# Gericom/MobiclipDecoder

Measured on AMD Instinct MI355X. Metric: decoded Mpixels/s @ 640x480 P-frames, higher is better.
Workload: dtype u8

## Files before the change

### mobiclipdecoder_amd/csrc/mobi_kernels.hip

```cpp
#include <hip/hip_runtime.h>
#include <stdint.h>
#include <stdlib.h>

#include <type_traits>

#include "mobi_cmd.h"
#include "mobi_kernels.h"
#include "mobi_recon_math.h"
#include "mobi_tile.h"

namespace {

enum { TP = 32 };

__device__ __forceinline__ void wave_sync() { __builtin_amdgcn_fence(__ATOMIC_ACQ_REL, "wavefront"); }

struct Geo {
  int width, height, stride, mbw, lg;
  __device__ __forceinline__ int owner_luma(int a) const {
    if (a < 0) return -1;
    const int row = a >> lg, col = a & (stride - 1);
    if (col >= width || row >= height) return -1;
    return (row >> 4) * mbw + (col >> 4);
  }
// ... 121 lines not shown
#else
#define MOBI_STOP(n) do { } while (0)
#define MOBI_ISTOP(n) do { } while (0)
#endif
namespace {
typedef const void __attribute__((address_space(1))) *gptr_t;
typedef void __attribute__((address_space(3))) *lptr_t;
#define MOBI_DMA16(src, dst, IMM) __builtin_amdgcn_global_load_lds((gptr_t)(src), (lptr_t)(dst), 16, IMM, 0)
__device__ __forceinline__ void dma16_sv(const uint8_t *base, uint32_t voff, uint32_t lds) {
#if defined(__HIP_DEVICE_COMPILE__)
  asm volatile("s_mov_b32 m0, %2\n\ts_nop 0\n\tglobal_load_lds_dwordx4 %0, %1" : : "v"(voff), "s"(base), "s"(lds) : "memory", "m0");
#endif
}

__device__ __forceinline__ uint32_t lds32(const uint8_t *L, int byte_off) { return *(const uint32_t *)(L + byte_off); }
typedef short s16x2 __attribute__((ext_vector_type(2)));
__device__ __forceinline__ uint32_t sat_pk_u8(s16x2 v) {
#if defined(__HIP_DEVICE_COMPILE__)
  uint32_t d;
  asm("v_sat_pk_u8_i16 %0, %1" : "=v"(d) : "v"(v));
  return d;
#else
  const int a = v.x < 0 ? 0 : v.x > 255 ? 255 : v.x, b = v.y < 0 ? 0 : v.y > 255 ? 255 : v.y;
  return (uint32_t)a | ((uint32_t)b << 8);
#endif
}
__device__ __forceinline__ void idct_pass2_q(const int *t, bool is8, int r, uint8_t *wa, uint8_t *wb, s16x2 &lo, s16x2 &hi) {
  int in[8], out[8];
  if (is8) {
#pragma unroll
    for (int m = 0; m < 8; m++) in[m] = t[8 * r + m];
    mobi_bfly8(in, out);
  } else {
    const int s = r >> 1, i0 = (r & 1) * 2;
#pragma unroll
    for (int m = 0; m < 8; m++) in[m] = t[16 * s + 4 * i0 + m];
    mobi_bfly4(in, out);
    mobi_bfly4(in + 4, out + 4);
  }
  const uint32_t pw[2] = {*(const uint32_t *)wa, *(const uint32_t *)wb};
  uint32_t res[2];
#pragma unroll
  for (int h = 0; h < 2; h++) {
    union { s16x2 v; uint32_t u; } p01, p23;
    p01.u = __builtin_amdgcn_perm(0u, pw[h], 0x0c010c00u);
    p23.u = __builtin_amdgcn_perm(0u, pw[h], 0x0c030c02u);
    const s16x2 r01 = __builtin_amdgcn_cvt_pk_i16(out[4 * h], out[4 * h + 1]) >> (short)6, r23 = __builtin_amdgcn_cvt_pk_i16(out[4 * h + 2], out[4 * h + 3]) >> (short)6;
    const s16x2 s01 = __builtin_elementwise_add_sat(p01.v, r01), s23 = __builtin_elementwise_add_sat(p23.v, r23);
    lo = __builtin_elementwise_min(lo, __builtin_elementwise_min(s01, s23));
    hi = __builtin_elementwise_max(hi, __builtin_elementwise_max(s01, s23));
    res[h] = __builtin_amdgcn_perm(sat_pk_u8(s23), sat_pk_u8(s01), 0x05040100u);
  }
  *(uint32_t *)wa = res[0];
  *(uint32_t *)wb = res[1];
}
}

#define MOBI_PK_LIMIT 14000
namespace {
__device__ __forceinline__ void bfly8_pk(const s16x2 in[8], s16x2 out[8]) {
  const s16x2 a0 = in[0] + in[4], a1 = in[0] - in[4];
  const s16x2 a2 = in[2] + (in[6] >> (short)1), a3 = (in[2] >> (short)1) - in[6];
  const s16x2 e0 = a0 + a2, e1 = a1 + a3, e2 = a1 - a3, e3 = a0 - a2;
  const s16x2 b0 = in[1] + in[7] - in[3] - (in[3] >> (short)1);
  const s16x2 b1 = in[7] - in[1] + in[5] + (in[5] >> (short)1);
  const s16x2 b2 = in[5] - (in[7] + (in[7] >> (short)1)) - in[3];
  const s16x2 b3 = in[3] + in[5] + in[1] + (in[1] >> (short)1);
  const s16x2 o0 = b2 + (b3 >> (short)2), o3 = b3 - (b2 >> (short)2);
  const s16x2 o1 = b0 + (b1 >> (short)2), o2 = (b0 >> (short)2) - b1;
  out[0] = e0 + o3; out[7] = e0 - o3;
  out[1] = e1 + o2; out[6] = e1 - o2;
  out[2] = e2 + o1; out[5] = e2 - o1;
  out[3] = e3 + o0; out[4] = e3 - o0;
}
__device__ __forceinline__ void bfly4_pk(const s16x2 in[4], s16x2 out[4]) {
  const s16x2 a = in[0] + in[2], b = in[0] - in[2];
  const s16x2 c = (in[1] >> (short)1) - in[3], d = in[1] + (in[3] >> (short)1);
  out[0] = a + d; out[3] = a - d; out[1] = b + c; out[2] = b - c;
}
union PkRow { uint4 q[2]; s16x2 v[8]; };
__device__ __forceinline__ void idct_pass1_pk(uint32_t *c, bool is8, int r) {
  PkRow in;
  s16x2 out[8];
  in.q[0] = *(const uint4 *)(c + 8 * r);
  in.q[1] = *(const uint4 *)(c + 8 * r + 4);
  const s16x2 rnd = {32, 32};
  if (is8) {
    if (r == 0) in.v[0] += rnd;
    bfly8_pk(in.v, out);
    wave_sync();
#pragma unroll
    for (int m = 0; m < 8; m++) *(s16x2 *)(c + 8 * m + r) = out[m];
  } else {
    const int s = r >> 1, k0 = (r & 1) * 2;
    if (k0 == 0) in.v[0] += rnd;
    bfly4_pk(in.v, out);
    bfly4_pk(in.v + 4, out + 4);
    wave_sync();
#pragma unroll
    for (int m = 0; m < 4; m++) *(uint2 *)(c + 16 * s + 4 * m + k0) = uint2{__builtin_bit_cast(uint32_t, out[m]), __builtin_bit_cast(uint32_t, out[4 + m])};
  }
}
__device__ __forceinline__ void idct_pass2_pk(const uint32_t *t, bool is8, int r, uint8_t *waA, uint8_t *wbA, uint8_t *waB, uint8_t *wbB, bool actB,
                                              s16x2 &lo, s16x2 &hi) {
  PkRow in;
  s16x2 out[8];
  in.q[0] = *(const uint4 *)(t + 8 * r);
  in.q[1] = *(const uint4 *)(t + 8 * r + 4);
  if (is8) {
    bfly8_pk(in.v, out);
  } else {
    bfly4_pk(in.v, out);
    bfly4_pk(in.v + 4, out + 4);
  }
  const uint32_t pA[2] = {*(const uint32_t *)waA, *(const uint32_t *)wbA}, pB[2] = {*(const uint32_t *)waB, *(const uint32_t *)wbB};
  uint32_t resA[2], resB[2];
#pragma unroll
  for (int h = 0; h < 2; h++) {
    uint32_t sat[4];
#pragma unroll
    for (int k = 0; k < 4; k++) {
      const s16x2 pp = __builtin_bit_cast(s16x2, __builtin_amdgcn_perm(pB[h], pA[h], 0x0c040c00u + (uint32_t)k * 0x00010001u));
      const s16x2 sum = __builtin_elementwise_add_sat(pp, out[4 * h + k] >> (short)6);
      lo = __builtin_elementwise_min(lo, sum);
      hi = __builtin_elementwise_max(hi, sum);
      sat[k] = sat_pk_u8(sum);
    }
    const uint32_t m01 = __builtin_amdgcn_perm(sat[1], sat[0], 0x05010400u), m23 = __builtin_amdgcn_perm(sat[3], sat[2], 0x05010400u);
    resA[h] = __builtin_amdgcn_perm(m23, m01, 0x05040100u);
    resB[h] = __builtin_amdgcn_perm(m23, m01, 0x07060302u);
  }
  *(uint32_t *)waA = resA[0];
  *(uint32_t *)wbA = resA[1];
  if (actB) {
    *(uint32_t *)waB = resB[0];
    *(uint32_t *)wbB = resB[1];
  }
}
}

namespace {
enum {
  P_L = 0,
  P_C = 5120,
  P_C1 = 7680,
  P_BYTES = 10240,
  P_OUT = 0,
  P_PITCH = 400,
  P_COEF = 3200,
  P_TILE = 72,
#ifndef MOBI_PK_PAIRS
#define MOBI_PK_PAIRS 12
#endif
  P_PAIRS = MOBI_PK_PAIRS,
  P_ROUND = 22,
  P_SUM = P_COEF + P_PAIRS * P_TILE * 4,
  P_SC = 9728,
  P_TAB = 10048,
  P_INV = 9536
};
static_assert(P_OUT + 7 * P_PITCH + 384 <= P_COEF && P_COEF + P_ROUND * P_TILE * 4 <= P_INV && P_INV + 192 <= P_SC && P_SC + 320 <= P_TAB && P_TAB + 192 <= P_BYTES && P_SUM + 192 <= P_INV, "inter LDS map");
static_assert(23 * P_TILE * 4 + 2 < (1 << 13) && (P_PITCH & 15) == 0, "P_INV's offset field (48 slots); 16-byte reads of the output rows");
__device__ __forceinline__ int out_px(int g, int R, int c) { return P_OUT + (R & 7) * P_PITCH + (R >> 3) * 128 + (g << 4) + c; }
__device__ __forceinline__ int out_y(int g, int R, int c) { return out_px(g, R, c); }
__device__ __forceinline__ int out_c(int g, int R, int pl, int x) { return out_px(g, 16 + R, pl * 8 + x); }
template <int N>
__device__ __forceinline__ void mc_rows(const uint32_t (&x0)[N + 1], const uint32_t (&x1)[N + 1], uint32_t sh, int phase, uint32_t *out) {
  const bool hor = (phase & 1) != 0, ver = (phase & 2) != 0;
  const uint32_t selA = 0x03020100u + sh * 0x01010101u, selB = hor ? selA + 0x01010101u : selA;
  const uint32_t Mh = hor ? 0xFEFEFEFEu : 0xFFFFFFFFu, Mv = ver ? 0xFEFEFEFEu : 0xFFFFFFFFu;
  uint32_t m[N + 1];
#pragma unroll
  for (int i = 0; i <= N; i++) {
    const uint32_t a = __builtin_amdgcn_perm(x1[i], x0[i], selA) & Mh, b = __builtin_amdgcn_perm(x1[i], x0[i], selB) & Mh;
    m[i] = __builtin_amdgcn_lerp(a, b, 0u) & Mv;
  }
#pragma unroll
  for (int i = 0; i < N; i++) out[i] = __builtin_amdgcn_lerp(m[i], ver ? m[i + 1] : m[i], 0u);
}
}

__device__ __forceinline__ unsigned long long prof_stamp() {
  __builtin_amdgcn_sched_barrier(0);
  asm volatile("" ::: "memory");
  const unsigned long long t = __builtin_readcyclecounter();
  asm volatile("" ::: "memory");
  __builtin_amdgcn_sched_barrier(0);
  return t;
}
template <int PROF, int CWR, int FUSED>
__device__ __forceinline__ void recon_inter_oct(const MobiReconArgs &A, uint8_t *L, uint32_t clip, uint32_t mby, uint32_t ox, int lane) {
  unsigned long long pt[7] = {0, 0, 0, 0, 0, 0, 0};
  if (PROF) pt[0] = prof_stamp();
  const uint32_t oi = clip * A.qpc + mby * A.qpr + ox;
  const uint32_t mbx0 = ox * 8, mbw = (uint32_t)A.mbw;
  const int nmb = (int)(mbw - mbx0 < 8 ? mbw - mbx0 : 8);
  const int S = A.stride, lgS = 31 - __builtin_clz((unsigned)S);
  const uint32_t ysz = (uint32_t)S * (uint32_t)A.height;
  uint8_t *clip_base = A.planes + (size_t)clip * A.clip_bytes;
  const uint32_t lds0 = (uint32_t)(size_t)(lptr_t)L;
  const int off0 = (int)(mby * 16 * (uint32_t)S + mbx0 * 16);
  const int g = lane & 7, j = lane >> 3;
  unsigned long long pa = 0, pb = 0;
  if (PROF) { asm volatile("" : : "s"(off0), "s"(clip)); pa = prof_stamp(); }

  __builtin_amdgcn_s_setprio(3);
  const uint4 *dp = (const uint4 *)(A.desc + (clip * (uint32_t)A.n_mbs + mby * mbw + mbx0) + g);
  const uint4 d = dp[0], d2 = dp[1];
  if (PROF) { asm volatile("s_waitcnt vmcnt(0)" ::: "memory"); pb = prof_stamp(); }
  const bool valid = g < nmb && (d.y & 1) == MOBI_MB_INTER;
  const int nl = (d.y >> 1) & 0x7F, kind2 = (d.y >> 26) & 3;
  const bool leaves = valid && (nl == 1 || kind2 != 0);
  const bool multi = valid && nl > 1 && kind2 == 0;
  const bool tb = leaves && kind2 == MOBI_DUAL_TB, lr = leaves && kind2 == MOBI_DUAL_LR;
  const uint32_t cbp6 = valid ? (d.y >> 8) & 0x3F : 0, ncoef = cbp6 ? d.z & 0x3FF : 0;
  const unsigned long long v64 = __builtin_amdgcn_ballot_w64(g < nmb) & __builtin_amdgcn_ballot_w64((d.y & 1) == MOBI_MB_INTER);
  const unsigned long long six = 0x0000FFFFFFFFFFFFull;
  const unsigned long long mb64 = __builtin_amdgcn_ballot_w64(((d.y >> (8 + j)) & 1) != 0) & v64 & six;
  const unsigned long long tb64 = __builtin_amdgcn_ballot_w64(((d.y >> (14 + j)) & 1) != 0) & six;
  const uint32_t m_lo = (uint32_t)mb64, m_hi = (uint32_t)(mb64 >> 32), t_lo = (uint32_t)tb64, t_hi = (uint32_t)(tb64 >> 32);
  const uint32_t inter_mask = (uint32_t)v64 & 0xFFu;
  const uint32_t multi_mask = (uint32_t)(v64 & __builtin_amdgcn_ballot_w64(nl > 1) & __builtin_amdgcn_ballot_w64(kind2 == 0)) & 0xFFu;
  if (inter_mask == 0) return;
  auto slot_off = [&](uint32_t ref) {
    int sl = A.ring_base - (int)ref;
    sl = sl < 0 ? sl + 6 : sl;
    return __umul24((uint32_t)sl, A.slot_bytes);
  };
  const uint32_t refA = slot_off((d.z >> 10) & 7), refB = slot_off((d.z >> 13) & 7);
  const int posA = (int)d.w, cposA = (int)d2.x, posB = (int)d2.y, cposB = (int)d2.z;
  const int phA = (d.z >> 16) & 3, cphA = (d.z >> 18) & 3, phB = (d.z >> 20) & 3, cphB = (d.z >> 22) & 3;
  const int topB = tb ? posB + (8 << lgS) : posB + 8, ctopB = tb ? cposB + (4 << lgS) : cposB + 4;
  const int wpx = lr ? 8 : 16, cwpx = lr ? 4 : 8;
  const int overA = max((posA & (S - 1)) + wpx + (phA & 1) - S, (cposA & (S - 1)) + cwpx + (cphA & 1) - (S >> 1));
  const int overB = max((topB & (S - 1)) + wpx + (phB & 1) - S, (ctopB & (S - 1)) + cwpx + (cphB & 1) - (S >> 1));
  const bool wrap = leaves && max(overA, kind2 != 0 ? overB : 0) > 0;
  const bool win = leaves && !wrap;
  const bool slow = multi || wrap;
  const uint32_t slow_mask = (uint32_t)__builtin_amdgcn_ballot_w64(slow) & 0xFFu;
  const bool any_lr = __builtin_amdgcn_ballot_w64(lr && win) != 0;
  {
    const int s = j & 3, ph = j >> 2;
    const bool colB = lr && s >= 2;
    const int sw = lr ? s & 1 : (s < 3 ? s : 2);
    auto chunk0 = [&](int top, uint32_t ref, uint32_t &u) {
      const int yo = (top >> lgS) & 1;
      const uint32_t lin = (uint32_t)(((top - (yo << lgS)) & ~7) + 8 * sw);
      u = lin >> (lgS + 1);
      return ref + mobi_ty_col(lin & (uint32_t)(S - 1));
    };
    uint32_t uP, uB;
    const uint32_t bP = chunk0(colB ? topB : posA, colB ? refB : refA, uP), bB = chunk0(topB, refB, uB);
    auto rowpart = [&](uint32_t v) { return ((v & ~7u) << (lgS + 1)) + (((v & 7u) + (v & 4u)) << 4); };
    const uint32_t Tm = (16u << lgS) - 256u;
    auto rows3 = [&](uint32_t base, uint32_t v, uint32_t (&r)[3]) {
      uint32_t h = (v >> 2) & 1u, e = (v >> 1) & 1u;
      asm volatile("" : "+v"(h), "+v"(e));
      const uint32_t dm = __umul24(h, Tm) + 64u;
      r[0] = base + rowpart(v);
      r[1] = __umul24(e, dm) + r[0] + 32u;
      r[2] = r[0] + 64u + dm;
    };
    const uint32_t vP = uP + (uint32_t)ph;
    uint32_t r1[3], r2[3];
    rows3(bP, vP, r1);
    rows3(tb ? bB : bP, tb ? uB + 1u - (uint32_t)ph : vP + 4u, r2);
    const bool early = tb && !ph;
    const bool short2 = tb != (ph != 0);
    const uint32_t o[5] = {r1[0], r1[1], early ? r1[2] : r2[0], early ? r2[0] : r2[1], short2 ? r2[1] : r2[2]};
    if (win) {
#pragma unroll
      for (int t = 0; t < 5; t++) dma16_sv(clip_base, o[t], lds0 + P_L + t * 1024);
    }
    const int cs = j & 1, ch2 = j >> 1;
    auto cchunk0 = [&](int ctop, uint32_t ref, uint32_t &r) {
      const uint32_t lin = (uint32_t)((ctop & ~7) + 8 * cs);
      r = lin >> lgS;
      return ref + ysz + mobi_tc_x(lin & (uint32_t)(S - 1));
    };
    auto crowpart = [&](uint32_t r) { return ((r & ~7u) << lgS) + ((r & 7u) << 4); };
    uint32_t rA, rB;
    const uint32_t cA = cchunk0(cposA, refA, rA), cB = cchunk0(ctopB, refB, rB);
    const uint32_t Tc = 8u << lgS, Tcm = Tc - 128u;
    auto cstep4 = [&](uint32_t r) {
      uint32_t h = (r >> 2) & 1u;
      asm volatile("" : "+v"(h));
      return __umul24(h, Tcm) + 64u;
    };
    const uint32_t qA = rA + (uint32_t)ch2;
    const uint32_t c0 = cA + crowpart(qA), cE = c0 + cstep4(qA);
    const uint32_t cY = cB + crowpart(rB + (uint32_t)((ch2 + 3) & 3));
    const uint32_t stB = cstep4(rB);
    const uint32_t cYd = cY + (ch2 == 1 ? stB : 0u);
    const uint32_t co[3] = {c0, (tb && ch2) ? cY : cE, tb ? cYd : (ch2 ? cE : c0 + Tc)};
    if (win) {
#pragma unroll
      for (int t = 0; t < 3; t++) dma16_sv(clip_base, co[t], lds0 + P_C + t * 1024);
    }
    if (any_lr) {
      const uint32_t q3 = rB + (uint32_t)ch2;
      if (lr && win) {
        const uint32_t z0 = cB + crowpart(q3), z1 = z0 + cstep4(q3);
        dma16_sv(clip_base, z0, lds0 + P_C1);
        dma16_sv(clip_base, z1, lds0 + P_C1 + 1024);
        dma16_sv(clip_base, ch2 ? z1 : z0 + Tc, lds0 + P_C1 + 2048);
      }
    }
  }
  MOBI_STOP(1);
  const int quant = __builtin_amdgcn_readfirstlane((int)((d.y >> 20) & 63));
  const uint32_t *pay = A.payload + (size_t)clip * A.pay_clip_words;
  const uint32_t *cw = pay + d.x + (multi ? MOBI_MV_CELLS : 0);
  uint32_t cwr[CWR];
#pragma unroll
  for (int k = 0; k < CWR; k++) asm volatile("" : "=v"(cwr[k]));
  const uint32_t *cwj = cw + j;
  const int left = (int)ncoef - j;
  if (left > 0) cwr[0] = cwj[0];
  if (__builtin_amdgcn_ballot_w64(ncoef > 8) != 0) {
#pragma unroll
    for (int k = 1; k < 4; k++)
      if (left > 8 * k) cwr[k] = cwj[8 * k];
    if (CWR > 4 && __builtin_amdgcn_ballot_w64(ncoef > 32) != 0) {
#pragma unroll
      for (int k = 4; k < CWR; k++)
        if (left > 8 * k) cwr[k] = cwj[8 * k];
    }
  }
  const int yrow = lane >> 2, yc4 = (lane & 3) * 4;
  const int cv = (lane >> 4) & 1, crow = (lane & 15) >> 1, cc4 = (lane & 1) * 4;
  uint32_t cell0 = 0, cell1 = 0;
  auto load_cell = [&](int gm, uint32_t &c) {
    if ((multi_mask >> gm) & 1) c = (pay + __builtin_amdgcn_readlane(d.x, gm))[lane];
  };
  if (slow_mask) {
    load_cell(__builtin_ctz(slow_mask), cell0);
    const uint32_t m2 = slow_mask & (slow_mask - 1);
    if (m2) load_cell(__builtin_ctz(m2), cell1);
  }
  if (PROF) pt[1] = prof_stamp();
  MOBI_STOP(2);
  asm volatile("s_waitcnt vmcnt(0)" ::: "memory");
  wave_sync();
  if (PROF) pt[2] = prof_stamp();

  struct Deep {
    bool cells;
    uint2 yr[3], ur[2], vr[2];
    uint32_t ysh, csh;
    int yph, cph;
    Win wa, wq;
    int pha, phq;
  };
  auto deep_fetch = [&](Deep &D, int gm, uint32_t cell) {
    const int offm = off0 + gm * 16;
    D.cells = (multi_mask >> gm) & 1;
    if (D.cells) {
      const int cy = lane >> 3, cx = lane & 7;
      const int dx = mobi_cell_dx(cell), dy = mobi_cell_dy(cell), qx = dx >> 1, qy = dy >> 1;
      const uint32_t sl = slot_off((uint32_t)mobi_cell_ref(cell));
      const int lo = offm + ((2 * cy + (dy >> 1)) << lgS) + 2 * cx + (dx >> 1);
      const int co = (offm >> 1) + ((cy + (qy >> 1)) << lgS) + cx + (qx >> 1);
      D.yph = (dx & 1) | ((dy & 1) << 1);
      D.cph = (qx & 1) | ((qy & 1) << 1);
      D.ysh = (uint32_t)lo & 3;
      D.csh = (uint32_t)co & 3;
      const uint32_t l4 = (uint32_t)lo & ~3u, c4 = (uint32_t)co & ~3u;
      const bool gen = (l4 & (uint32_t)(S - 1)) >= (uint32_t)(S - 8) || (c4 & (uint32_t)(S - 1)) >= (uint32_t)((S >> 1) - 8);
      if (__builtin_amdgcn_ballot_w64(gen) != 0) {
#pragma unroll
        for (int k = 0; k < 3; k++) {
          D.yr[k].x = *(const uint32_t *)(clip_base + (sl + mobi_ty(l4 + (uint32_t)(k << lgS), lgS)));
          D.yr[k].y = *(const uint32_t *)(clip_base + (sl + mobi_ty(l4 + (uint32_t)(k << lgS) + 4, lgS)));
        }
#pragma unroll
        for (int k = 0; k < 2; k++) {
          const uint32_t a0 = sl + ysz + mobi_tc(c4 + (uint32_t)(k << lgS), lgS), a1 = sl + ysz + mobi_tc(c4 + (uint32_t)(k << lgS) + 4, lgS);
          const uint32_t b0 = sl + ysz + mobi_tc(c4 + (uint32_t)(k << lgS) + (uint32_t)(S >> 1), lgS), b1 = sl + ysz + mobi_tc(c4 + (uint32_t)(k << lgS) + (uint32_t)(S >> 1) + 4, lgS);
          D.ur[k] = uint2{*(const uint32_t *)(clip_base + a0), *(const uint32_t *)(clip_base + a1)};
          D.vr[k] = uint2{*(const uint32_t *)(clip_base + b0), *(const uint32_t *)(clip_base + b1)};
        }
      } else {
        const uint32_t t = sl + mobi_ty(l4, lgS), row = l4 >> lgS;
        const uint32_t dc = (l4 & 4u) ? ((l4 & 8u) ? 188u : 60u) : 4u;
        auto down = [&](uint32_t r) { return (r & 7u) != 7u ? 8u : (r & 8u) ? ((16u << lgS) - 184u) : 72u; };
        const uint32_t t1 = t + down(row), t2 = t1 + down(row + 1);
        D.yr[0] = uint2{*(const uint32_t *)(clip_base + t), *(const uint32_t *)(clip_base + (t + dc))};
        D.yr[1] = uint2{*(const uint32_t *)(clip_base + t1), *(const uint32_t *)(clip_base + (t1 + dc))};
        D.yr[2] = uint2{*(const uint32_t *)(clip_base + t2), *(const uint32_t *)(clip_base + (t2 + dc))};
        const uint32_t u = sl + ysz + mobi_tc(c4, lgS), crow0 = c4 >> lgS;
        const uint32_t cdc = (c4 & 4u) ? 124u : 4u, cdr = (crow0 & 7u) != 7u ? 16u : (8u << lgS) - 112u;
        D.ur[0] = uint2{*(const uint32_t *)(clip_base + u), *(const uint32_t *)(clip_base + (u + cdc))};
        D.vr[0] = uint2{*(const uint32_t *)(clip_base + (u + 8)), *(const uint32_t *)(clip_base + (u + cdc + 8))};
        D.ur[1] = uint2{*(const uint32_t *)(clip_base + (u + cdr)), *(const uint32_t *)(clip_base + (u + cdr + cdc))};
        D.vr[1] = uint2{*(const uint32_t *)(clip_base + (u + cdr + 8)), *(const uint32_t *)(clip_base + (u + cdr + cdc + 8))};
      }
    } else {
      const uint32_t w1m = __builtin_amdgcn_readlane(d.y, gm), w2m = __builtin_amdgcn_readlane(d.z, gm);
      const int pAm = (int)__builtin_amdgcn_readlane(d.w, gm), cAm = (int)__builtin_amdgcn_readlane(d2.x, gm);
      const int pBm = (int)__builtin_amdgcn_readlane(d2.y, gm), cBm = (int)__builtin_amdgcn_readlane(d2.z, gm);
      const int k2 = (w1m >> 26) & 3;
      const bool yBm = k2 == MOBI_DUAL_TB ? yrow >= 8 : k2 == MOBI_DUAL_LR ? yc4 >= 8 : false;
      const bool cBl2 = k2 == MOBI_DUAL_TB ? crow >= 4 : k2 == MOBI_DUAL_LR ? cc4 >= 4 : false;
      const int la = (yBm ? pBm : pAm) + (yrow << lgS) + yc4;
      D.pha = (w2m >> (yBm ? 20 : 16)) & 3;
      const uint32_t sa = slot_off((w2m >> (yBm ? 13 : 10)) & 7);
      const int lq = (cBl2 ? cBm : cAm) + cv * (S >> 1) + (crow << lgS) + cc4;
      D.phq = (w2m >> (cBl2 ? 22 : 18)) & 3;
      const uint32_t sq = slot_off((w2m >> (cBl2 ? 13 : 10)) & 7);
      const bool gen = (((uint32_t)la & (uint32_t)(S - 1)) >= (uint32_t)(S - 8)) || (((uint32_t)lq & (uint32_t)((S >> 1) - 1)) >= (uint32_t)((S >> 1) - 8));
      const bool general = __builtin_amdgcn_ballot_w64(gen) != 0;
      D.wa = fetch_win_y(clip_base, sa, la, S, lgS, general);
      D.wq = fetch_win_c(clip_base, sq + ysz, lq, S, lgS, general);
    }
  };
  auto deep_finish = [&](int gm, const Deep &D) {
    if (D.cells) {
      const int cy = lane >> 3, cx = lane & 7;
      const uint32_t M = 0x7F7F7F7Fu;
      uint32_t a[3], h[3];
#pragma unroll
      for (int k = 0; k < 3; k++) {
        a[k] = cut(D.yr[k], D.ysh);
        const uint32_t b = cut1(D.yr[k], D.ysh);
        h[k] = ((a[k] >> 1) & M) + ((b >> 1) & M);
      }
      uint32_t yo[2];
#pragma unroll
      for (int k = 0; k < 2; k++) {
        const uint32_t v = ((a[k] >> 1) & M) + ((a[k + 1] >> 1) & M), p3 = ((h[k] >> 1) & M) + ((h[k + 1] >> 1) & M);
        yo[k] = D.yph == 0 ? a[k] : D.yph == 1 ? h[k] : D.yph == 2 ? v : p3;
      }
      *(uint16_t *)(L + out_y(gm, 2 * cy, 2 * cx)) = (uint16_t)yo[0];
      *(uint16_t *)(L + out_y(gm, 2 * cy + 1, 2 * cx)) = (uint16_t)yo[1];
      const uint32_t au = cut(D.ur[0], D.csh), bu = cut1(D.ur[0], D.csh), cu = cut(D.ur[1], D.csh), du = cut1(D.ur[1], D.csh);
      const uint32_t av = cut(D.vr[0], D.csh), bv = cut1(D.vr[0], D.csh), cvv = cut(D.vr[1], D.csh), dv = cut1(D.vr[1], D.csh);
      const uint32_t ca = __builtin_amdgcn_perm(av, au, 0x0c0c0400u), cb = __builtin_amdgcn_perm(bv, bu, 0x0c0c0400u);
      const uint32_t cc = __builtin_amdgcn_perm(cvv, cu, 0x0c0c0400u), cd = __builtin_amdgcn_perm(dv, du, 0x0c0c0400u);
      const uint32_t hca = (ca >> 1) & M, hcb = (cb >> 1) & M, hcc = (cc >> 1) & M, hcd = (cd >> 1) & M;
      const uint32_t c1 = hca + hcb, c2 = hca + hcc, c3 = ((c1 >> 1) & M) + (((hcc + hcd) >> 1) & M);
      const uint32_t uvp = D.cph == 0 ? ca : D.cph == 1 ? c1 : D.cph == 2 ? c2 : c3;
      L[out_c(gm, cy, 0, cx)] = (uint8_t)uvp;
      L[out_c(gm, cy, 1, cx)] = (uint8_t)(uvp >> 8);
    } else {
      const uint32_t va = mc4_select(D.wa, D.pha), cpred = mc4_select(D.wq, D.phq);
      *(uint32_t *)(L + out_y(gm, yrow, yc4)) = va;
      if (lane < 32) *(uint32_t *)(L + out_c(gm, crow, cv, cc4)) = cpred;
    }
  };
  Deep D0;
  if (slow_mask) deep_fetch(D0, __builtin_ctz(slow_mask), cell0);

  __builtin_amdgcn_s_setprio(0);
  MOBI_STOP(3);
  uint32_t mcv[12];
  const int rr = j >> 2, q = j & 3;
  const int pl = j >> 2, ch = (j >> 1) & 1, qc = j & 1;
  {
    const bool cBl = (tb && ch) || (lr && qc);
    const int ctop = cBl ? ctopB : cposA, cph = cBl ? cphB : cphA;
    const int cxo = ctop & 7, d0 = (cxo + (lr ? 0 : 4 * qc)) >> 2, d1 = d0 + 1;
    const int base = ((lr && qc) ? P_C1 : P_C) + ((tb && ch) ? 5 : 4 * ch) * 256 + g * 16 + pl * 8;
    const int a0 = base + (d0 >> 1) * 128 + (d0 & 1) * 4, a1 = base + (d1 >> 1) * 128 + (d1 & 1) * 4;
    uint32_t x0[5], x1[5];
#pragma unroll
    for (int k = 0; k < 5; k++) { x0[k] = lds32(L, a0 + k * 256); x1[k] = lds32(L, a1 + k * 256); }
    mc_rows<4>(x0, x1, (uint32_t)cxo & 3u, cph, mcv + 8);
  }
  MOBI_STOP(4);
  asm volatile("s_waitcnt lgkmcnt(0)" ::: "memory");
  if (lane < MOBI_SCALE_STRIDE / 4) MOBI_DMA16((const uint8_t *)(A.scale + quant * MOBI_SCALE_STRIDE) + lane * 16, L + P_SC, 0);
  {
    const bool rB = tb && rr, qB = lr && q >= 2;
    const int ytop = rB || qB ? topB : posA, yph = rB || qB ? phB : phA;
    const int yo = (ytop >> lgS) & 1, xo = ytop & 7;
    const int d0 = (xo + 4 * (qB ? q - 2 : q)) >> 2, d1 = d0 + 1;
    const int base = P_L + (rB ? 5 : 4 * rr) * 512 + g * 16 + (qB ? 256 : 0);
    const int a0 = base + (d0 >> 1) * 128 + (d0 & 1) * 4, a1 = base + (d1 >> 1) * 128 + (d1 & 1) * 4;
    const int ev = yo * 8, od = yo ? 512 : 8;
    uint32_t x0[9], x1[9];
#pragma unroll
    for (int k = 0; k < 9; k++) {
      const int o = (k >> 1) * 512 + ((k & 1) ? od : ev);
      x0[k] = lds32(L, a0 + o);
      x1[k] = lds32(L, a1 + o);
    }
    mc_rows<8>(x0, x1, (uint32_t)xo & 3u, yph, mcv);
  }
  MOBI_STOP(5);
  wave_sync();
  {
    const int by = out_y(g, 8 * rr, 4 * q), bc = out_c(g, 4 * ch, pl, 4 * qc);
#pragma unroll
    for (int k = 0; k < 8; k++) *(uint32_t *)(L + (by + k * P_PITCH)) = mcv[k];
#pragma unroll
    for (int k = 0; k < 4; k++) *(uint32_t *)(L + (bc + k * P_PITCH)) = mcv[8 + k];
  }
  if (PROF) pt[3] = prof_stamp();
  MOBI_STOP(6);
  if (slow_mask) {
    asm volatile("s_waitcnt vmcnt(0)" ::: "memory");
    deep_finish(__builtin_ctz(slow_mask), D0);
    uint32_t mm = slow_mask & (slow_mask - 1);
    bool second = true;
    while (mm) {
      const int gm = __builtin_ctz(mm);
      mm &= mm - 1;
      uint32_t cell = cell1;
      if (!second) load_cell(gm, cell);
      second = false;
      Deep Dn;
      deep_fetch(Dn, gm, cell);
      asm volatile("" ::: "memory");
      deep_finish(gm, Dn);
    }
  }
  if (PROF) pt[4] = prof_stamp();
  MOBI_STOP(7);

  asm volatile("s_waitcnt vmcnt(0)" ::: "memory");
  wave_sync();
  if (m_lo | m_hi) {
    const uint32_t m8_lo = m_lo & t_lo, m8_hi = m_hi & t_hi, m4_lo = m_lo & ~t_lo, m4_hi = m_hi & ~t_hi;
    const int n8_lo = __builtin_popcount(m8_lo), n8 = n8_lo + __builtin_popcount(m8_hi);
    const int n4_lo = __builtin_popcount(m4_lo), first4 = (n8 + 1) & ~1, n_slots = first4 + n4_lo + __builtin_popcount(m4_hi);
    {
      const bool hi = lane >= 32;
      const int kk = lane & 31;
      if (((hi ? m_hi : m_lo) >> kk) & 1) {
        const bool is8 = ((hi ? t_hi : t_lo) >> kk) & 1;
        const uint32_t flip = is8 ? 0u : 0xFFFFFFFFu;
        const uint32_t mask = hi ? m_hi & (t_hi ^ flip) : m_lo & (t_lo ^ flip);
        const int first = (is8 ? 0 : first4) + (hi ? (is8 ? n8_lo : n4_lo) : 0);
        const int slot = first + __builtin_popcount(mask & ((1u << kk) - 1u));
        const int a = lane >> 3;
        const uint32_t K = (uint32_t)((a < 4 ? a >> 1 : 2) * 128 + (a & 1) * 8);
        *(uint32_t *)(L + P_TAB + 4 * slot) = ((uint32_t)lane << 8) | ((K + ((uint32_t)(lane & 7) << 4)) << 16);
        *(uint32_t *)(L + P_INV + 4 * lane) = (uint32_t)((slot >> 1) * (P_TILE * 4) + (slot & 1) * 2) | ((uint32_t)slot << 13) | ((is8 ? 0x0FCu : 0x13Cu) << 23);
      }
      if (lane < 48) *(uint32_t *)(L + P_SUM + 4 * lane) = 0u;
    }
    wave_sync();
    MOBI_STOP(8);
    s16x2 lo = {0, 0}, hi = {0, 0};
    const int r = lane & 7, grp = lane >> 3;
    auto scatter_all = [&](auto pk, int base) {
      constexpr bool PK = decltype(pk)::value;
      const int base_off = PK ? (base >> 1) * (P_TILE * 4) : 0;
      auto scatter = [&](uint32_t e) {
        const uint32_t t = e & 0x1FF, t4 = t << 2, p4 = t4 & 0xFCu, kk4 = ((t >> 6) * 8 + (uint32_t)g) << 2;
        const int level = (int32_t)e >> 16;
        const uint32_t inv = lds32(L, P_INV + (int)kk4);
        const int scale = (int)lds32(L, P_SC + (int)((t4 | 0x100u) & (inv >> 23)));
        const int v = __mul24(scale, level);
        if (PK) {
          const uint32_t off = (inv & 0x1FFFu) - (uint32_t)base_off;
          if (off < (uint32_t)(P_PAIRS * P_TILE * 4)) *(int16_t *)(L + P_COEF + off + p4) = (int16_t)v;
          if (base == 0) {
            const int av = v < 0 ? -v : v;
            __hip_atomic_fetch_add((uint32_t *)(L + P_SUM + kk4), (uint32_t)(av > 0xFFFF ? 0xFFFF : av), __ATOMIC_RELAXED, __HIP_MEMORY_SCOPE_WAVEFRONT);
          }
        } else {
          const int slot = (int)((inv >> 13) & 0x7Fu) - base;
          if ((unsigned)slot < (unsigned)P_ROUND) *(int *)(L + P_COEF + slot * (P_TILE * 4) + p4) = v;
        }
      };
#pragma unroll
      for (int k = 0; k < CWR; k++) {
        int lf = left;
        asm volatile("" : "+v"(lf));
        const bool mine = lf > 8 * k;
        if (k && __builtin_amdgcn_ballot_w64(mine) == 0) break;
        uint32_t e = cwr[k];
        asm volatile("" : "+v"(e));
        if (mine) scatter(e);
      }
      for (uint32_t i = 8u * CWR + (uint32_t)j; __builtin_amdgcn_ballot_w64(i < ncoef) != 0; i += 64) {
        uint32_t tw[8];
#pragma unroll
        for (int k = 0; k < 8; k++) tw[k] = i + 8u * k < ncoef ? cw[i + 8u * k] : 0u;
#pragma unroll
        for (int k = 0; k < 8; k++)
          if (i + 8u * k < ncoef) scatter(tw[k]);
      }
    };
    auto zero_tiles = [&](int n_tiles) {
      const uint4 z = uint4{0, 0, 0, 0};
      for (int o = lane * 16; o < n_tiles * P_TILE * 4; o += 1024) *(uint4 *)(L + P_COEF + o) = z;
    };
    const int s4 = r >> 1, rowa4 = (s4 >> 1) * 4 + (r & 1) * 2, cola4 = (s4 & 1) * 4;
    const int Ca8 = P_OUT + r * P_PITCH, Ca4 = P_OUT + rowa4 * P_PITCH + cola4;
    bool wide = false;
    for (int base = 0; base < n_slots && !wide; base += 2 * P_PAIRS) {
      zero_tiles(n_slots - base < 2 * P_PAIRS ? (n_slots - base + 1) >> 1 : P_PAIRS);
      wave_sync();
      scatter_all(std::true_type{}, base);
      wave_sync();
      if (base == 0) {
        const uint32_t sm = lane < 48 ? lds32(L, P_SUM + 4 * lane) : 0u;
        if (__builtin_amdgcn_ballot_w64(sm > (uint32_t)MOBI_PK_LIMIT) != 0) { wide = true; break; }
      }
      MOBI_STOP(9);
      for (int sub = 0; sub < P_PAIRS && base + 2 * sub < n_slots; sub += 8) {
        const int slot0 = base + 2 * (sub + grp);
        const bool act = sub + grp < P_PAIRS && slot0 < n_slots, is8g = slot0 < first4;
        const bool actB = slot0 + 1 < n_slots && slot0 + 1 != n8;
        uint32_t *tile = (uint32_t *)(L + P_COEF) + P_TILE * (sub + grp);
        if (act) idct_pass1_pk(tile, is8g, r);
        wave_sync();
        MOBI_STOP(10);
        if (act) {
          const uint32_t recA = lds32(L, P_TAB + 4 * slot0), recB = actB ? lds32(L, P_TAB + 4 * slot0 + 4) : recA;
          const int Ca = is8g ? Ca8 : Ca4, dab = is8g ? 4 : P_PITCH;
          uint8_t *wa = L + (Ca + (int)(recA >> 16)), *wb = wa + dab, *wc = L + (Ca + (int)(recB >> 16)), *wd = wc + dab;
          idct_pass2_pk(tile, is8g, r, wa, wb, wc, wd, actB, lo, hi);
        }
        wave_sync();
        MOBI_STOP(11);
      }
    }
    if (wide) {
      const int hole = (n8 & 1) ? n8 : -1;
      for (int base = 0; base < n_slots; base += P_ROUND) {
        zero_tiles(n_slots - base < P_ROUND ? n_slots - base : P_ROUND);
        wave_sync();
        scatter_all(std::false_type{}, base);
        wave_sync();
        int *coef = (int *)(L + P_COEF);
        uint32_t recx[3];
        bool actx[3], is8x[3];
#pragma unroll
        for (int h = 0; h < 3; h++) {
          const int idx = base + 8 * h + grp;
          actx[h] = idx < n_slots && idx != hole && 8 * h + grp < P_ROUND;
          recx[h] = actx[h] ? lds32(L, P_TAB + 4 * idx) : 0u;
          is8x[h] = idx < n8;
        }
#pragma unroll
        for (int h = 0; h < 3; h++) {
          int *tile = coef + P_TILE * (8 * h + grp);
          if (actx[h]) idct_pass1(tile, tile, is8x[h], r);
        }
        wave_sync();
#pragma unroll
        for (int h = 0; h < 3; h++) {
          if (actx[h]) {
            const bool is8 = is8x[h];
            uint8_t *wa = L + ((is8 ? Ca8 : Ca4) + (int)(recx[h] >> 16));
            idct_pass2_q(coef + P_TILE * (8 * h + grp), is8, r, wa, wa + (is8 ? 4 : P_PITCH), lo, hi);
          }
        }
        wave_sync();
      }
    }
    if (lo.x < -64 || lo.y < -64 || hi.x > 319 || hi.y > 319) atomicOr(&A.fault[clip], 1);
  }
  if (PROF) { asm volatile("s_waitcnt lgkmcnt(0)" ::: "memory"); pt[5] = prof_stamp(); }

  MOBI_STOP(12);
  __builtin_amdgcn_s_setprio(3);
  {
    uint8_t *y0 = clip_base + (uint32_t)A.ring_base * A.slot_bytes;
    uint8_t *ty0 = y0 + mobi_tile_y(mbx0, mby, lgS), *tc0 = y0 + ysz + mobi_tile_c(mbx0, mby, lgS);
    const bool full = nmb == 8;
    if (FUSED) {
#pragma unroll
      for (int it = 0; it < 2; it++) {
        const int i = lane + 64 * it, gq = i >> 4, quad = (i >> 2) & 3, R0 = (quad >> 1) * 8 + 2 * (i & 3), c0 = (quad & 1) * 8;
        const uint2 v0 = *(const uint2 *)(L + out_y(gq, R0, c0)), v1 = *(const uint2 *)(L + out_y(gq, R0 + 1, c0));
        const u32x4 v = {v0.x, v0.y, v1.x, v1.y};
        const uint8_t *dst = ty0 + i * 16;
        if ((inter_mask >> gq) & 1) asm volatile("global_store_dwordx4 %0, %1, off sc1\n\ts_nop 1" : : "v"(dst), "v"(v) : "memory");
      }
      {
        const int gq = lane >> 3, R = lane & 7;
        const uint4 c4 = *(const uint4 *)(L + out_c(gq, R, 0, 0));
        const u32x4 vc = {c4.x, c4.y, c4.z, c4.w};
        const uint8_t *dst = tc0 + lane * 16;
        if ((inter_mask >> gq) & 1) asm volatile("global_store_dwordx4 %0, %1, off sc1\n\ts_nop 1" : : "v"(dst), "v"(vc) : "memory");
      }
      asm volatile("s_waitcnt vmcnt(0)" ::: "memory");
      if (lane < 8 && ((inter_mask >> lane) & 1))
        __hip_atomic_store(A.done + (size_t)clip * A.n_mbs + mby * mbw + mbx0 + lane, A.step_tag, __ATOMIC_RELAXED, __HIP_MEMORY_SCOPE_AGENT);
    } else {
#pragma unroll
    for (int it = 0; it < 2; it++) {
      const int i = lane + 64 * it, gq = i >> 4, quad = (i >> 2) & 3, R0 = (quad >> 1) * 8 + 2 * (i & 3), c0 = (quad & 1) * 8;
      const uint2 v0 = *(const uint2 *)(L + out_y(gq, R0, c0)), v1 = *(const uint2 *)(L + out_y(gq, R0 + 1, c0));
      if (full) *(uint4 *)(ty0 + i * 16) = uint4{v0.x, v0.y, v1.x, v1.y};
      else *(uint4 *)(ty0 + i * 16) = gq < nmb ? uint4{v0.x, v0.y, v1.x, v1.y} : uint4{0, 0, 0, 0};
    }
    {
      const int gq = lane >> 3, R = lane & 7;
      const uint4 vc = *(const uint4 *)(L + out_c(gq, R, 0, 0));
      if (full) *(uint4 *)(tc0 + lane * 16) = vc;
      else *(uint4 *)(tc0 + lane * 16) = gq < nmb ? vc : uint4{0, 0, 0, 0};
    }
    }
  }
  if (PROF && lane == 0) {
    pt[6] = prof_stamp();
    unsigned long long *rec = A.prof + (size_t)oi * 8;
#pragma unroll
    for (int k = 0; k < 6; k++) rec[k] = pt[k + 1] - pt[k];
    rec[6] = 1ull | ((pa - pt[0]) << 8) | ((pb - pa) << 32);
    rec[7] = (unsigned long long)(__builtin_popcount(m_lo) + __builtin_popcount(m_hi));
  }
}
#define MOBI_OCT_KERNEL(NAME, WAVES, PROF, NCWR)                                                      \
  extern "C" __global__ __launch_bounds__(64, WAVES) void NAME(MobiReconArgs A) {                      \
    __shared__ __attribute__((aligned(16))) uint8_t lds[P_BYTES];                                      \
    const uint32_t oi = (blockIdx.x & 7) * A.inter_per_xcd + (blockIdx.x >> 3);                        \
    if (oi >= A.qpc * (uint32_t)A.n_clips) return;                                                     \
    uint32_t rem, ox;                                                                                  \
    const uint32_t clip = fastdiv(oi, A.qpc, A.magic_qpc, rem);  \
    const uint32_t mby = fastdiv(rem, A.qpr, A.magic_qpr, ox);                                         \
    recon_inter_oct<PROF, NCWR, 0>(A, lds, clip, mby, ox, (int)threadIdx.x);                              \
  }
MOBI_OCT_KERNEL(mobi_recon_inter8, 4, 0, 16)
#if defined(MOBI_PROFILING)
MOBI_OCT_KERNEL(mobi_recon_inter8_prof, 4, 1, 16)
#endif

namespace {
enum { IQ_TILE = 768,
       IQ_TCU = 17 * TP, IQ_TCV = IQ_TCU + 9 * TP,
       IQ_SCALE = 1536 / 4, IQ_WORDS = (IQ_TILE + IQ_TCV + 9 * TP) / 4,
       IQ_TAB = 1856 };
static_assert(IQ_WORDS * 4 == 1888 && IQ_SCALE * 4 + 320 <= IQ_TAB && IQ_TAB + 24 <= IQ_WORDS * 4 && 4 * IQ_WORDS * 4 <= 6 * 1280, "intra LDS map");
__device__ __forceinline__ int step_word(int k) { const int row = (k * 43) >> 7; return IQ_TILE + IQ_TCU + row * TP + 20 + 4 * (k - 3 * row); }
enum { SD_O = 0,
       SD_TAP = 11,
       SD_IS4 = 1 << 21,
       SD_CODED = 1 << 22,
       SD_KTAP = 1 << 23, SD_KDC = 1 << 24, SD_KPLANE = 1 << 25,
       SD_TA = 1 << 26, SD_LA = 1 << 27,
       SD_P4 = 1 << 30 };

__device__ __forceinline__ uint32_t ldg_u8_sc1(const uint8_t *p) {
  uint32_t v = 0;
#if defined(__HIP_DEVICE_COMPILE__)
  asm volatile("global_load_ubyte %0, %1, off sc1" : "=v"(v) : "v"(p) : "memory");
#endif
  return v;
}
__device__ __forceinline__ uint32_t tap_addr(uint32_t base, uint32_t packed, int hi) {
  uint32_t d = 0;
#if defined(__HIP_DEVICE_COMPILE__)
  if (hi) asm("v_add_u32_sdwa %0, %1, sext(%2) dst_sel:DWORD dst_unused:UNUSED_PAD src0_sel:DWORD src1_sel:WORD_1" : "=v"(d) : "v"(base), "v"(packed));
// ... 606 lines not shown
```

Measured before the change: 1.042 million.

## Batch the first coefficient scatter pass and prefetch later macroblock descriptors

When all slots fit in one packed round, the coefficient scatter now runs in batches: it issues several LDS reads of the inverse table and scale table before doing the multiplies and stores, which hides LDS latency. The batch size depends on the wave-wide coefficient count. It also adds a dummy global load of a descriptor about 1024 macroblocks ahead in the non-fused path, to warm the cache for later workgroups. This adds code size and register pressure. Lanes with no coefficient word now do speculative LDS reads, which the added static_assert checks stay in bounds.

```diff
diff --git a/mobiclipdecoder_amd/csrc/mobi_kernels.hip b/mobiclipdecoder_amd/csrc/mobi_kernels.hip
--- a/mobiclipdecoder_amd/csrc/mobi_kernels.hip
+++ b/mobiclipdecoder_amd/csrc/mobi_kernels.hip
@@ -297,6 +297,7 @@
 #ifndef MOBI_PK_PAIRS
 #define MOBI_PK_PAIRS 12
 #endif
+  P_TOUCH = 1024,
   P_PAIRS = MOBI_PK_PAIRS,
   P_ROUND = 22,
   P_SUM = P_COEF + P_PAIRS * P_TILE * 4,
@@ -305,6 +306,7 @@
   P_INV = 9536
 };
 static_assert(P_OUT + 7 * P_PITCH + 384 <= P_COEF && P_COEF + P_ROUND * P_TILE * 4 <= P_INV && P_INV + 192 <= P_SC && P_SC + 320 <= P_TAB && P_TAB + 192 <= P_BYTES && P_SUM + 192 <= P_INV, "inter LDS map");
+static_assert(P_INV + 4 * 63 < P_BYTES && P_SC + 0x1FC < P_BYTES, "what a lane without a word may read in a batch of the scatter");
 static_assert(23 * P_TILE * 4 + 2 < (1 << 13) && (P_PITCH & 15) == 0, "P_INV's offset field (48 slots); 16-byte reads of the output rows");
 __device__ __forceinline__ int out_px(int g, int R, int c) { return P_OUT + (R & 7) * P_PITCH + (R >> 3) * 128 + (g << 4) + c; }
 __device__ __forceinline__ int out_y(int g, int R, int c) { return out_px(g, R, c); }
@@ -352,6 +354,15 @@
   __builtin_amdgcn_s_setprio(3);
   const uint4 *dp = (const uint4 *)(A.desc + (clip * (uint32_t)A.n_mbs + mby * mbw + mbx0) + g);
   const uint4 d = dp[0], d2 = dp[1];
+  uint32_t touch = 0;
+  if (!FUSED) {
+    const uint32_t own = clip * (uint32_t)A.n_mbs + mby * mbw + mbx0, total = (uint32_t)A.n_clips * (uint32_t)A.n_mbs;
+    uint32_t room = max(total, 8u);
+    asm volatile("" : "+s"(room));
+    const uint32_t later = min(own + (uint32_t)P_TOUCH, room - 8u);
+    const uint8_t *tb = (const uint8_t *)A.desc + (size_t)later * sizeof(MbDesc);
+    touch = *(const uint32_t *)(tb + (uint32_t)lane * 4u);
+  }
   if (PROF) { asm volatile("s_waitcnt vmcnt(0)" ::: "memory"); pb = prof_stamp(); }
   const bool valid = g < nmb && (d.y & 1) == MOBI_MB_INTER;
   const int nl = (d.y >> 1) & 0x7F, kind2 = (d.y >> 26) & 3;
@@ -486,6 +497,7 @@
   if (PROF) pt[1] = prof_stamp();
   MOBI_STOP(2);
   asm volatile("s_waitcnt vmcnt(0)" ::: "memory");
+  if (!FUSED) asm volatile("" : : "v"(touch));
   wave_sync();
   if (PROF) pt[2] = prof_stamp();
 
@@ -689,10 +701,10 @@
     MOBI_STOP(8);
     s16x2 lo = {0, 0}, hi = {0, 0};
     const int r = lane & 7, grp = lane >> 3;
-    auto scatter_all = [&](auto pk, int base) {
+    auto scatter_one = [&](auto pk, int base, uint32_t e) {
       constexpr bool PK = decltype(pk)::value;
       const int base_off = PK ? (base >> 1) * (P_TILE * 4) : 0;
-      auto scatter = [&](uint32_t e) {
+      {
         const uint32_t t = e & 0x1FF, t4 = t << 2, p4 = t4 & 0xFCu, kk4 = ((t >> 6) * 8 + (uint32_t)g) << 2;
         const int level = (int32_t)e >> 16;
         const uint32_t inv = lds32(L, P_INV + (int)kk4);
@@ -709,7 +721,20 @@
           const int slot = (int)((inv >> 13) & 0x7Fu) - base;
           if ((unsigned)slot < (unsigned)P_ROUND) *(int *)(L + P_COEF + slot * (P_TILE * 4) + p4) = v;
         }
-      };
+      }
+    };
+    auto scatter_rest = [&](auto pk, int base) {
+      for (uint32_t i = 8u * CWR + (uint32_t)j; __builtin_amdgcn_ballot_w64(i < ncoef) != 0; i += 64) {
+        uint32_t tw[8];
+#pragma unroll
+        for (int k = 0; k < 8; k++) tw[k] = i + 8u * k < ncoef ? cw[i + 8u * k] : 0u;
+#pragma unroll
+        for (int k = 0; k < 8; k++)
+          if (i + 8u * k < ncoef) scatter_one(pk, base, tw[k]);
+      }
+    };
+    auto scatter_all = [&](auto pk, int base) {
+      auto scatter = [&](uint32_t e) { scatter_one(pk, base, e); };
 #pragma unroll
       for (int k = 0; k < CWR; k++) {
         int lf = left;
@@ -720,15 +745,61 @@
         asm volatile("" : "+v"(e));
         if (mine) scatter(e);
       }
-      for (uint32_t i = 8u * CWR + (uint32_t)j; __builtin_amdgcn_ballot_w64(i < ncoef) != 0; i += 64) {
-        uint32_t tw[8];
-#pragma unroll
-        for (int k = 0; k < 8; k++) tw[k] = i + 8u * k < ncoef ? cw[i + 8u * k] : 0u;
-#pragma unroll
-        for (int k = 0; k < 8; k++)
-          if (i + 8u * k < ncoef) scatter(tw[k]);
-      }
+      scatter_rest(pk, base);
     };
+    static_assert(CWR == 16, "scatter_first's batches: words 0 .. 127 in registers");
+    const int g4 = 4 * g;
+    auto batch = [&](auto k0c, auto bc) {
+      constexpr int K0 = decltype(k0c)::value, B = decltype(bc)::value;
+      uint32_t e[B], t4[B], kk[B], inv[B];
+      int sc[B];
+      int lf = left;
+      asm volatile("" : "+v"(lf));
+#pragma unroll
+      for (int i = 0; i < B; i++) {
+        e[i] = cwr[K0 + i];
+        asm volatile("" : "+v"(e[i]));
+        t4[i] = e[i] << 2;
+        kk[i] = (((e[i] >> 6) & 7u) << 5) + (uint32_t)g4;
+        inv[i] = lds32(L, P_INV + (int)kk[i]);
+      }
+#pragma unroll
+      for (int i = 0; i < B; i++) sc[i] = (int)lds32(L, P_SC + (int)((t4[i] | 0x100u) & (inv[i] >> 23)));
+      int v[B];
+      uint32_t at[B], av[B];
+#pragma unroll
+      for (int i = 0; i < B; i++) {
+        v[i] = __mul24(sc[i], (int32_t)e[i] >> 16);
+        at[i] = (inv[i] & 0x1FFFu) + (t4[i] & 0xFCu);
+        const int a = v[i] < 0 ? -v[i] : v[i];
+        av[i] = (uint32_t)(a > 0xFFFF ? 0xFFFF : a);
+        asm volatile("" : "+v"(v[i]), "+v"(at[i]), "+v"(av[i]));
+      }
+#pragma unroll
+      for (int i = 0; i < B; i++) {
+        if (lf > 8 * (K0 + i)) {
+          *(int16_t *)(L + P_COEF + at[i]) = (int16_t)v[i];
+          __hip_atomic_fetch_add((uint32_t *)(L + P_SUM + kk[i]), av[i], __ATOMIC_RELAXED, __HIP_MEMORY_SCOPE_WAVEFRONT);
+        }
+      }
+    };
+#define MOBI_BATCH(K0, B) batch(std::integral_constant<int, K0>{}, std::integral_constant<int, B>{})
+    auto scatter_first = [&]() {
+      if (__builtin_amdgcn_ballot_w64(ncoef > 16) == 0) MOBI_BATCH(0, 2);
+      else if (__builtin_amdgcn_ballot_w64(ncoef > 24) == 0) MOBI_BATCH(0, 3);
+      else {
+        MOBI_BATCH(0, 4);
+        if (__builtin_amdgcn_ballot_w64(ncoef > 32) != 0) {
+          if (CWR > 4) MOBI_BATCH(4, 4);
+          if (CWR > 8 && __builtin_amdgcn_ballot_w64(ncoef > 64) != 0) {
+            MOBI_BATCH(8, 4);
+            if (CWR > 12 && __builtin_amdgcn_ballot_w64(ncoef > 96) != 0) MOBI_BATCH(12, 4);
+          }
+          scatter_rest(std::true_type{}, 0);
+        }
+      }
+    };
+#undef MOBI_BATCH
     auto zero_tiles = [&](int n_tiles) {
       const uint4 z = uint4{0, 0, 0, 0};
       for (int o = lane * 16; o < n_tiles * P_TILE * 4; o += 1024) *(uint4 *)(L + P_COEF + o) = z;
@@ -739,7 +810,8 @@
     for (int base = 0; base < n_slots && !wide; base += 2 * P_PAIRS) {
       zero_tiles(n_slots - base < 2 * P_PAIRS ? (n_slots - base + 1) >> 1 : P_PAIRS);
       wave_sync();
-      scatter_all(std::true_type{}, base);
+      if (n_slots <= 2 * P_PAIRS) scatter_first();
+      else scatter_all(std::true_type{}, base);
       wave_sync();
       if (base == 0) {
         const uint32_t sm = lane < 48 ? lds32(L, P_SUM + 4 * lane) : 0u;
```

Measured after the change: 1.053 million (median of 6 runs). 1.0% higher.
